# UPC-ViRVIG/DragPoser

Hardware: AMD Instinct MI355X
Metric: frames/sec (6 trackers, 50 iters/frame) (higher is better)
Workload: dtype f32

## Files before the change

dragposer_amd/csrc/dp_w4_impl.h:

```cpp
#pragma once
#ifndef W4_BP
#define W4_BP 0
#endif
#ifndef W4_SKEL
#define W4_SKEL 0
#endif
#ifndef W4_KERNEL
#define W4_KERNEL dp_w4_kernel
#endif
#include "dp_device.h"
#include "dp_w4.h"
#include <utility>

using namespace dpw4;

template <class F, int... I> DEV void static_for_impl(F&& f, std::integer_sequence<int, I...>) { (f(std::integral_constant<int, I>{}), ...); }
template <int N, class F> DEV void static_for(F&& f) { static_for_impl(f, std::make_integer_sequence<int, N>{}); }

constexpr int W4_R = 24;
constexpr int FB_QS = 0;
constexpr int FB_BN = FB_QS + 128;
constexpr int FB_GP = FB_BN + 128;
constexpr int FB_RT = FB_GP + 4 * W4_R;
constexpr int FB_WT = FB_RT + 4 * W4_R;
// ... 297 lines not shown
};
static_assert(sizeof(StepArgs) <= L_ARGS_WORDS * 4 && alignof(StepArgs) <= 16, "StepArgs fits its LDS slot");
DEV void stage_step_args(float* lds, const KArgs& a)
{
    StepArgs* d = (StepArgs*)(lds + L_ARGS);
    d->items = a.items; d->w4img = a.w4img;
    d->z_tgt = a.z_tgt; d->tgt_pos = a.tgt_pos; d->tgt_rot = a.tgt_rot; d->w = a.w;
    d->z = a.z; d->z_pre = a.z_pre; d->pose = a.pose; d->disp = a.disp; d->world_disp = a.world_disp; d->world_rot = a.world_rot;
    d->pos = a.pos; d->rot = a.rot; d->loss = a.loss;
    d->iters = a.iters; d->status = a.status;
    d->n_iter = a.n_iter;
    d->lam_rot = a.lam_rot; d->lam_tmp = a.lam_tmp;
    d->seq = a.seq;
}
template <bool SEQ> DEV decltype(auto) step_args_of(const KArgs& a, const float* lds)
{
    if constexpr (SEQ) {
        int o = L_ARGS;
        asm volatile("" : "+v"(o));
        return *(const StepArgs*)(lds + o);
    } else {
        return (a);
    }
}

DEV int nth_set_bit(unsigned m, int rank)
{
    int pos = 0;
#pragma unroll
    for (int step = 16; step >= 1; step >>= 1) {
        const int c = __popc(m & ((1u << (pos + step)) - 1u));
        pos += c <= rank ? step : 0;
    }
    return pos;
}
struct TRaw {
    bool act;
    int rank, j;
    unsigned plo, phi;
    float p[3], wp, wr, m[9];
};
template <class A> DEV TRaw tracker_fetch(const A& a, bool optimise, int gf, unsigned tmask, int E, int rank, int gf_tgt = -1)
{
    TRaw r;
    r.act = rank < E;
    r.rank = rank;
    const int j = r.act ? nth_set_bit(tmask, rank) : 0;
    r.j = j;
    {
        const auto* it = (const dpl::ItemConst __attribute__((address_space(1)))*)a.items + j;
        r.plo = it->path_lo;
        r.phi = it->path_hi;
    }
    const int row = optimise ? gf * NJ + j : 0;
    const size_t rowt = optimise ? (size_t)(gf_tgt >= 0 ? gf_tgt : gf) * NJ + j : 0;
    const gfloat* p = GM(optimise ? a.tgt_pos : a.w4img) + rowt * 3;
    const gfloat* rm = GM(optimise ? a.tgt_rot : a.w4img) + rowt * 9;
    const gfloat* wv = GM(optimise ? a.w : a.w4img) + (size_t)row * 2;
    r.p[0] = p[0]; r.p[1] = p[1]; r.p[2] = p[2];
    r.wp = wv[0];
    r.wr = wv[1];
#pragma unroll
    for (int k = 0; k < 9; ++k) r.m[k] = rm[k];
    return r;
}
template <class A> DEV TRec tracker_finish(const A& a, float* fb, const TRaw& r, int E, Q4 cur, V3 shift = V3{0.f, 0.f, 0.f})
{
    TRec t;
    t.act = r.act;
    t.rank = r.rank;
    const int j = r.j;
    t.qs = FB_QS + 4 * (j == 0 ? QS_IDENT : j);
    t.wt = FB_WT + 4 * (j == 0 ? WT_TRASH : j);
    t.plo = r.plo;
    t.phi = r.phi;
    t.tp = {0.f, 0.f, 0.f};
    t.qT0 = f2{1.f, 0.f}; t.qT1 = f2{0.f, 0.f};
    t.cgp = t.clp = t.k8 = t.clr8 = 0.f;
    if (t.act) {
        const float invE = 1.f / (float)E;
        t.tp = rot_conj(cur, V3{r.p[0] + shift.x, r.p[1] + shift.y, r.p[2] + shift.z});
        const Q4 qT = quat_mul(Q4{cur.w, -cur.x, -cur.y, -cur.z}, quat_from_rotmat(r.m));
        t.qT0 = f2{qT.w, qT.x}; t.qT1 = f2{qT.y, qT.z};
        t.clp = r.wp * invE * (1.f / 3.f);
        const float clr = a.lam_rot * r.wr * invE * (1.f / 9.f);
        t.cgp = 2.f * t.clp;
        t.k8 = -8.f * clr;
        t.clr8 = 8.f * clr;
        float* ti = fb + FB_TI + r.rank * 4;
        *(f4*)(ti) = f4{t.tp.x, t.tp.y, t.tp.z, t.cgp};
        *(f4*)(ti + 4 * W4_R) = f4{qT.w, qT.x, qT.y, qT.z};
        *(f4*)(ti + 8 * W4_R) = f4{t.k8, t.clp, t.clr8, __int_as_float(j)};
    }
    return t;
}
DEV bool out_of_range(float x) { return !(fabsf(x) <= DP_INPUT_LIMIT); }
DEV bool raw_bad(const TRaw& r)
{
    bool bad = out_of_range(r.p[0]) || out_of_range(r.p[1]) || out_of_range(r.p[2]) || out_of_range(r.wp) || out_of_range(r.wr);
#pragma unroll
    for (int k = 0; k < 9; ++k) bad = bad || out_of_range(r.m[k]);
    return r.act && bad;
}
DEV void raw_neutral(TRaw& r)
{
    r.p[0] = r.p[1] = r.p[2] = 0.f;
    r.wp = r.wr = 0.f;
#pragma unroll
    for (int k = 0; k < 9; ++k) r.m[k] = (k % 4 == 0) ? 1.f : 0.f;
}
DEV unsigned frames_of(unsigned long long votes)
{
    votes |= votes >> 32; votes |= votes >> 16; votes |= votes >> 8; votes |= votes >> 4;
    return (unsigned)votes & 0xFu;
}
DEV float poisoned(bool p, float v) { return p ? __builtin_nanf("") : v; }
template <class A> DEV TRec make_tracker(const A& a, float* fb, int gf, unsigned tmask, int E, int rank, Q4 cur, int gf_tgt = -1, V3 shift = V3{0.f, 0.f, 0.f}, bool neutral = false)
{
    TRaw r = tracker_fetch(a, true, gf, tmask, E, rank, gf_tgt);
    if (neutral) raw_neutral(r);
    return tracker_finish(a, fb, r, E, cur, shift);
}

DEV TRec load_tracker(const KArgs& a, const float* fb, int E, int rank)
{
    TRec t;
    t.act = rank < E;
    t.rank = rank;
    const float* ti = fb + FB_TI + (t.act ? rank : 0) * 4;
    const f4 i0 = *(const f4*)(ti), i1 = *(const f4*)(ti + 4 * W4_R), i2 = *(const f4*)(ti + 8 * W4_R);
    const int j = t.act ? __float_as_int(i2.w) : 0;
    t.qs = FB_QS + 4 * (j == 0 ? QS_IDENT : j);
    t.wt = FB_WT + 4 * (j == 0 ? WT_TRASH : j);
    t.plo = a.items[j].path_lo;
    t.phi = a.items[j].path_hi;
    t.tp = {i0.x, i0.y, i0.z};
    t.cgp = i0.w;
    t.qT0 = f2{i1.x, i1.y}; t.qT1 = f2{i1.z, i1.w};
    t.k8 = i2.x; t.clp = i2.y; t.clr8 = i2.z;
    return t;
}

DEV void lds_store4(float* p, float a, float b, float c, float d)
{
    const unsigned ad = (unsigned)(size_t)p;
    asm volatile("ds_write2_b32 %0, %1, %2 offset1:1\n\tds_write2_b32 %0, %3, %4 offset0:2 offset1:3" : : "v"(ad), "v"(a), "v"(b), "v"(c), "v"(d) : "memory");
}
DEV void lds_store3(float* p, float a, float b, float c)
{
    const unsigned ad = (unsigned)(size_t)p;
    asm volatile("ds_write2_b32 %0, %1, %2 offset1:1\n\tds_write_b32 %0, %3 offset:8" : : "v"(ad), "v"(a), "v"(b), "v"(c) : "memory");
}

struct JOut { f2 q[4], u[3], inv; };
DEV void j_stage(const PairC& c, float* fb, const f4 y01, const f4 y23, JOut& o)
{
    const f2 rq[4] = {f2{y01[0], y01[1]}, f2{y01[2], y01[3]}, f2{y23[0], y23[1]}, f2{y23[2], y23[3]}};
    const f2 nn = rq[0] * rq[0] + rq[1] * rq[1] + rq[2] * rq[2] + rq[3] * rq[3];
#if W4_BP
    const float invA = c.kindA == KIND_DISP ? 1.f : (c.kindA == KIND_IDLE ? 0.f : __builtin_amdgcn_rsqf(nn.x));
    const float invB = c.kindB == KIND_IDLE ? 0.f : __builtin_amdgcn_rsqf(nn.y);
#else
    const float invA = __builtin_amdgcn_rsqf(nn.x);
    const float invB = c.kindB == KIND_DISP ? 1.f : (c.kindB == KIND_IDLE ? 0.f : __builtin_amdgcn_rsqf(nn.y));
#endif
    o.inv = f2{invA, invB};
#pragma unroll
    for (int k = 0; k < 4; ++k) o.q[k] = rq[k] * o.inv;
    const f2 w = o.q[0], vx = o.q[1], vy = o.q[2], vz = o.q[3];
    const f2 tx = vy * c.off[2] - vz * c.off[1], ty = vz * c.off[0] - vx * c.off[2], tz = vx * c.off[1] - vy * c.off[0];
    const f2 cx = vy * tz - vz * ty, cy = vz * tx - vx * tz, cz = vx * ty - vy * tx;
    o.u[0] = c.off[0] + 2.f * (w * tx + cx);
    o.u[1] = c.off[1] + 2.f * (w * ty + cy);
    o.u[2] = c.off[2] + 2.f * (w * tz + cz);
    lds_store4(fb + c.qsA, o.q[0].x, o.q[1].x, o.q[2].x, o.q[3].x);
    lds_store4(fb + c.qsB, o.q[0].y, o.q[1].y, o.q[2].y, o.q[3].y);
    lds_store3(fb + c.bnA, o.u[0].x, o.u[1].x, o.u[2].x);
    lds_store3(fb + c.bnB, o.u[0].y, o.u[1].y, o.u[2].y);
}

DEV void quat_mul_conj_a(f2 a0, f2 a1, f2 b0, f2 b1, f2& o0, f2& o1)
{
    asm("v_pk_mul_f32 %0, %2, %4 op_sel:[1,1] op_sel_hi:[1,0] neg_hi:[0,1]\n\t"
        "v_pk_mul_f32 %1, %2, %5 op_sel:[1,1] op_sel_hi:[1,0] neg_hi:[0,1]\n\t"
        "v_pk_fma_f32 %0, %2, %4, %0 op_sel_hi:[0,1,1]\n\t"
        "v_pk_fma_f32 %1, %2, %5, %1 op_sel_hi:[0,1,1]\n\t"
        "v_pk_fma_f32 %0, %3, %5, %0 op_sel_hi:[0,1,1] neg_hi:[0,1,0]\n\t"
        "v_pk_fma_f32 %1, %3, %4, %1 op_sel_hi:[0,1,1] neg_lo:[0,1,0]\n\t"
        "v_pk_fma_f32 %0, %3, %5, %0 op_sel:[1,1,0] op_sel_hi:[1,0,1]\n\t"
        "v_pk_fma_f32 %1, %3, %4, %1 op_sel:[1,1,0] op_sel_hi:[1,0,1] neg_lo:[0,1,0] neg_hi:[0,1,0]"
        : "=&v"(o0), "=&v"(o1)
        : "v"(a0), "v"(a1), "v"(b0), "v"(b1));
}
DEV void quat_mul_conj_b(f2 a0, f2 a1, f2 b0, f2 b1, f2& o0, f2& o1)
{
    asm("v_pk_mul_f32 %0, %2, %4 op_sel:[1,1] op_sel_hi:[1,0]\n\t"
        "v_pk_mul_f32 %1, %2, %5 op_sel:[1,1] op_sel_hi:[1,0] neg_hi:[0,1]\n\t"
        "v_pk_fma_f32 %0, %2, %4, %0 op_sel_hi:[0,1,1] neg_hi:[0,1,0]\n\t"
        "v_pk_fma_f32 %1, %2, %5, %1 op_sel_hi:[0,1,1] neg_lo:[0,1,0] neg_hi:[0,1,0]\n\t"
        "v_pk_fma_f32 %0, %3, %5, %0 op_sel_hi:[0,1,1] neg_hi:[0,1,0]\n\t"
        "v_pk_fma_f32 %1, %3, %4, %1 op_sel_hi:[0,1,1]\n\t"
        "v_pk_fma_f32 %0, %3, %5, %0 op_sel:[1,1,0] op_sel_hi:[1,0,1]\n\t"
        "v_pk_fma_f32 %1, %3, %4, %1 op_sel:[1,1,0] op_sel_hi:[1,0,1] neg_lo:[0,1,0]"
        : "=&v"(o0), "=&v"(o1)
        : "v"(a0), "v"(a1), "v"(b0), "v"(b1));
}

DEV void t_stage(const TRec& t, float* fb, bool losses)
{
    if (!t.act) return;
    const f4 q0v = *(const f4*)(fb + FB_QS), qtv = *(const f4*)(fb + t.qs), dv = *(const f4*)(fb + FB_QS + 4 * QS_DISP);
    f2 pxy = f2{dv.x, dv.y};
    float pz = dv.z;
    {
        const unsigned plo = t.plo, phi = t.phi;
        f4 bn[MAX_PATH];
#pragma unroll
        for (int k = 0; k < MAX_PATH; ++k) bn[k] = *(const f4*)(fb + FB_BN + 4 * ((k < 6) ? ((plo >> (5 * k)) & 31u) : (phi & 31u)));
#pragma unroll
        for (int k = 0; k < MAX_PATH; ++k) { pxy += f2{bn[k].x, bn[k].y}; pz += bn[k].z; }
    }
    const Q4 q0 = {q0v.x, q0v.y, q0v.z, q0v.w};
    const V3 at = rot_conj(q0, t.tp);
    const f2 exy = pxy - f2{at.x, at.y};
    const float ez = pz - at.z;
    const f2 gpxy = t.cgp * exy;
    const float gpz = t.cgp * ez;
    const V3 e = {exy.x, exy.y, ez}, gp = {gpxy.x, gpxy.y, gpz};
    f2 r0, r1, s0, s1;
    quat_mul_conj_a(f2{q0v.x, q0v.y}, f2{q0v.z, q0v.w}, t.qT0, t.qT1, r0, r1);
    quat_mul_conj_b(r0, r1, f2{qtv.x, qtv.y}, f2{qtv.z, qtv.w}, s0, s1);
    const Q4 s = {s0.x, s0.y, s1.x, s1.y};
    const float k = t.k8 * s.w;
    const float ownx = k * s.x;
    const f2 ownyz = k * s1;
    const V3 own = {ownx, ownyz.x, ownyz.y};
    const V3 ag = cross(at, gp);
    const f2 rtyz = f2{ag.y, ag.z} + ownyz;
    const V3 rt = {ag.x + own.x, rtyz.x, rtyz.y};
    typedef float f3 __attribute__((ext_vector_type(3)));
    *(f3*)(fb + FB_GP + 4 * t.rank) = f3{gp.x, gp.y, gp.z};
    *(f3*)(fb + FB_RT + 4 * t.rank) = f3{rt.x, rt.y, rt.z};
    *(f3*)(fb + t.wt) = f3{own.x, own.y, own.z};
    if (losses)
        *(f2*)(fb + FB_LP + 2 * t.rank) = f2{t.clp * (e.x * e.x + e.y * e.y + e.z * e.z), t.clr8 * (s.x * s.x + s.y * s.y + s.z * s.z)};
}

DEV void g_stage(const PairC& c, const float* fb, const JOut& j, unsigned tmask, int Emax, f4& gyA, f4& gyB)
{
    f2 S[3] = {splat2(0.f), splat2(0.f), splat2(0.f)};
    {
        const float* tab = fb + c.tab;
        f4 g[6];
#pragma unroll
        for (int u = 0; u < 6; ++u) g[u] = *(const f4*)(tab + 4 * u);
#pragma unroll
        for (int u = 0; u < 6; ++u) asm volatile("" : "+v"(g[u]));
#pragma unroll
        for (int u = 0; u < 6; ++u) { S[0] += c.sel[u] * splat2(g[u].x); S[1] += c.sel[u] * splat2(g[u].y); S[2] += c.sel[u] * splat2(g[u].z); }
        if (Emax > 6) {
            unsigned m = tmask;
#pragma unroll
            for (int u = 0; u < 6; ++u) m &= m - 1u;
            for (int e0 = 6; e0 < Emax; ++e0) {
                const f4 ge = *(const f4*)(tab + 4 * e0);
                const int t = __builtin_ctz(m | 0x80000000u);
                m &= m - 1u;
                const f2 sl = f2{(float)((c.subA >> t) & 1u), (float)((c.subB >> t) & 1u)};
                S[0] += sl * splat2(ge.x); S[1] += sl * splat2(ge.y); S[2] += sl * splat2(ge.z);
            }
        }
    }
    f4 wa = *(const f4*)(fb + c.wtA), wb = *(const f4*)(fb + c.wtB);
    asm volatile("" : "+v"(wa), "+v"(wb));
    f2 t0 = j.u[1] * S[2] - j.u[2] * S[1] + c.rho * S[0];
    f2 t1 = j.u[2] * S[0] - j.u[0] * S[2] + c.rho * S[1];
    f2 t2 = j.u[0] * S[1] - j.u[1] * S[0] + c.rho * S[2];
    t0.x += wa.x; t0.y += wb.x; t1.x += wa.y; t1.y += wb.y; t2.x += wa.z; t2.y += wb.z;
    const f2 a0 = t0 + t0, a1 = t1 + t1, a2 = t2 + t2;
    const f2 w = j.q[0], vx = j.q[1], vy = j.q[2], vz = j.q[3];
    const f2 g0 = -(a0 * vx + a1 * vy + a2 * vz);
    const f2 g1 = w * a0 + c.sgn * (a1 * vz - a2 * vy);
    const f2 g2 = w * a1 + c.sgn * (a2 * vx - a0 * vz);
    const f2 g3 = w * a2 + c.sgn * (a0 * vy - a1 * vx);
    const f2 si = j.inv;
    f2 y0 = g0 * si, y1 = g1 * si, y2 = g2 * si, y3 = g3 * si;
#if W4_BP
    if (c.kindA == KIND_DISP) { y0.x = S[0].x; y1.x = S[1].x; y2.x = S[2].x; y3.x = 0.f; }
#else
    if (c.kindB == KIND_DISP) { y0.y = S[0].y; y1.y = S[1].y; y2.y = S[2].y; y3.y = 0.f; }
#endif
    gyA = f4{y0.x, y1.x, y2.x, y3.x};
    gyB = f4{y0.y, y1.y, y2.y, y3.y};
}

struct OutC { int item, kind; f4 sd, mu; unsigned plo, phi; };
DEV void out_consts(const float* oc, int itemA, int kindA, int itemB, int kindB, OutC& oA, OutC& oB)
{
    const f4* t = (const f4*)oc;
    const f4 s0 = t[0], s1 = t[1], m0 = t[2], m1 = t[3], pw = t[4];
    oA.item = itemA; oA.kind = kindA;
    oB.item = itemB; oB.kind = kindB;
    oA.sd = f4{s0.x, s0.z, s1.x, s1.z}; oB.sd = f4{s0.y, s0.w, s1.y, s1.w};
    oA.mu = f4{m0.x, m0.z, m1.x, m1.z}; oB.mu = f4{m0.y, m0.w, m1.y, m1.w};
    oA.plo = __float_as_uint(pw.x); oA.phi = __float_as_uint(pw.y);
    oB.plo = __float_as_uint(pw.z); oB.phi = __float_as_uint(pw.w);
}
template <bool SEQ = false, class A>
DEV void w4_outputs(const A& a, const OutC& oc, float* fb, int gf, bool optimise, Q4 cur, unsigned tmask, bool early, bool pall = false, bool ploss = false)
{
    const int item = oc.item, kind = oc.kind;
    const auto P = [pall](float v) { return poisoned(pall, v); };
    if (item < 0 || kind == KIND_IDLE || kind == KIND_VIRT) return;
    const f4 sd = oc.sd, mu = oc.mu;
    const f4 qv = *(const f4*)(fb + FB_QS + 4 * item);
    const Q4 rq = {qv.x, qv.y, qv.z, qv.w};
    const f4 q0v = *(const f4*)(fb + FB_QS);
    const Q4 qw = quat_mul(cur, Q4{q0v.x, q0v.y, q0v.z, q0v.w});
    const M3 R0 = quat_to_mat(qw);
    if (kind == KIND_DISP) {
        if (a.disp) { gfloat* o = GM(a.disp) + (size_t)gf * 3; o[0] = P(rq.w); o[1] = P(rq.x); o[2] = P(rq.y); }
        if (a.world_disp || SEQ) {
            const V3 wd = mat_vec(R0, V3{rq.w, rq.x, rq.y});
            if (a.world_disp) { gfloat* o = GM(a.world_disp) + (size_t)gf * 3; o[0] = P(wd.x); o[1] = P(wd.y); o[2] = P(wd.z); }
            if (SEQ) { *(f4*)(fb + FB_SWD) = f4{wd.x, wd.y, wd.z, 0.f}; *(f4*)(fb + FB_SD) = f4{rq.w, rq.x, rq.y, 0.f}; }
        }
        return;
    }
    const Q4 q = rq;
    if (a.pose) {
        gfloat* o = GM(a.pose) + (size_t)gf * 88 + 4 * item;
        if (SEQ && kind == KIND_ROOT) {
            o[0] = P((qw.w - a.seq.mean_q0[0]) / a.seq.std_q0[0]); o[1] = P((qw.x - a.seq.mean_q0[1]) / a.seq.std_q0[1]);
            o[2] = P((qw.y - a.seq.mean_q0[2]) / a.seq.std_q0[2]); o[3] = P((qw.z - a.seq.mean_q0[3]) / a.seq.std_q0[3]);
        } else {
            o[0] = P((q.w - mu.x) / sd.x); o[1] = P((q.x - mu.y) / sd.y); o[2] = P((q.y - mu.z) / sd.z); o[3] = P((q.z - mu.w) / sd.w);
        }
    }
    if (a.pos || SEQ) {
        const f4 dv = *(const f4*)(fb + FB_QS + 4 * QS_DISP);
        V3 pr = {dv.x, dv.y, dv.z};
        const unsigned plo = oc.plo, phi = oc.phi;
        f4 bn[MAX_PATH];
#pragma unroll
        for (int k = 0; k < MAX_PATH; ++k) bn[k] = *(const f4*)(fb + FB_BN + 4 * ((k < 6) ? ((plo >> (5 * k)) & 31u) : (phi & 31u)));
#pragma unroll
        for (int k = 0; k < MAX_PATH; ++k) { pr.x += bn[k].x; pr.y += bn[k].y; pr.z += bn[k].z; }
        const V3 pw = mat_vec(R0, pr);
        if (a.pos) { gfloat* o = GM(a.pos) + ((size_t)gf * NJ + item) * 3; o[0] = P(pw.x); o[1] = P(pw.y); o[2] = P(pw.z); }
        if (SEQ) { float* o = fb + FB_SPOS + 3 * item; o[0] = pw.x; o[1] = pw.y; o[2] = pw.z; }
    }
    if (a.rot) {
        M3 M = quat_to_mat(q);
        if (kind == KIND_ROOT) M = {1.f, 0.f, 0.f, 0.f, 1.f, 0.f, 0.f, 0.f, 1.f};
        const M3 G = mat_mat(R0, M);
        gfloat* o = GM(a.rot) + ((size_t)gf * NJ + item) * 9;
        o[0] = P(G.m00); o[1] = P(G.m01); o[2] = P(G.m02); o[3] = P(G.m10); o[4] = P(G.m11); o[5] = P(G.m12); o[6] = P(G.m20); o[7] = P(G.m21); o[8] = P(G.m22);
    }
    if (kind == KIND_ROOT) {
        if (a.world_rot) { gfloat* o = GM(a.world_rot) + (size_t)gf * 4; o[0] = P(qw.w); o[1] = P(qw.x); o[2] = P(qw.y); o[3] = P(qw.z); }
        if (SEQ) *(f4*)(fb + FB_SQW) = f4{qw.w, qw.x, qw.y, qw.z};
        if (optimise && a.loss && early) {
            const f4 es = *(const f4*)(fb + FB_ES);
            gfloat* o = GM(a.loss) + (size_t)gf * 3;
            o[0] = poisoned(ploss, es.x); o[1] = poisoned(ploss, es.y); o[2] = poisoned(ploss, es.z);
        } else if (optimise && a.loss) {
            float lsum_p = 0.f, lsum_r = 0.f, lt = 0.f;
            const int E = min(__popc(tmask), W4_R);
            for (int e0 = 0; e0 < E; ++e0) { const f2 l = *(const f2*)(fb + FB_LP + 2 * e0); lsum_p += l.x; lsum_r += l.y; }
            for (int k = 0; k < LAT; k += 4) {
                const f4 dz = *(const f4*)(fb + FB_ZPRE + k) - *(const f4*)(fb + FB_ZT + k);
                lt += dz.x * dz.x + dz.y * dz.y + dz.z * dz.z + dz.w * dz.w;
            }
            gfloat* o = GM(a.loss) + (size_t)gf * 3;
            o[0] = poisoned(ploss, lsum_p);
            o[1] = poisoned(ploss, lsum_r);
            o[2] = poisoned(ploss, lt * a.lam_tmp * (1.f / 24.f));
        }
    }
}

#ifndef W4_B2_RES_A
#define W4_B2_RES_A 3
#endif
#ifndef W4_B2_RES_V
#define W4_B2_RES_V 2
#endif
#ifndef W4_B2_RES_A_SEQ
#define W4_B2_RES_A_SEQ 1
#endif
template <int NW, bool EARLY, bool SEQ = false, bool LONG = false>
__global__ __launch_bounds__(NW * 64, 1) void W4_KERNEL(const KArgs a)
{
    static_assert(!SEQ || EARLY, "sequences run the reference's while-condition");
    static_assert(W4_B2_RES_A_SEQ >= 1 && W4_B2_RES_A >= 1, "the first resident group of bL2 starts the chain from zero");
    __shared__ __attribute__((aligned(16))) float lds[lds_total<NW>()];

#ifdef DP_PROFILE
    const unsigned long long t_entry = __builtin_amdgcn_s_memtime();
    unsigned long long t_setup[5] = {0, 0, 0, 0, 0};
#define SETUP_STAMP(i) do { __builtin_amdgcn_sched_barrier(0); t_setup[i] = __builtin_amdgcn_s_memtime(); __builtin_amdgcn_sched_barrier(0); } while (0)
#else
#define SETUP_STAMP(i)
#endif
    const int tid = threadIdx.x;
    const int lane = tid & 63;
    const int wave = __builtin_amdgcn_readfirstlane(tid >> 6);
    const int b = lane >> 2, i = lane & 3;
    const int nB = a.n_frames;
    const int f0 = (blockIdx.x * NW + wave) * FPW;
    const bool optimise = (a.mode == 0);

    const int gfi = min(f0 + i, nB - 1);
    const bool fvalid = f0 + i < nB;
    float* fb0 = lds + L_FR + wave * FPW * FB_STRIDE;
    float* fb = fb0 + i * FB_STRIDE;

    constexpr int N_IMG = N_GROUPS * 64, N_LD = (N_IMG + NW * 64 - 1) / (NW * 64);
    static_assert((N_GROUPS - NG_B2) * 256 <= lds_total<NW>() - L_TAB, "the staging area holds the resident groups");
    f4 im[N_LD];
#pragma unroll
    for (int k = 0; k < N_LD; ++k)
        if (tid + k * NW * 64 < N_IMG) im[k] = ((const f4*)a.w4img)[tid + k * NW * 64];
    __builtin_amdgcn_sched_barrier(0);

    typedef unsigned u32_any __attribute__((aligned(1), may_alias));
// ... 253 lines not shown
    const bool clk_on = a.clk != nullptr && blockIdx.x == 0 && wave == 0;
    unsigned long long clk_c0 = 0, clk_r0 = 0;
    if (clk_on) { clk_r0 = __builtin_amdgcn_s_memrealtime(); clk_c0 = __builtin_amdgcn_s_memtime(); }
    int step = 0;
#ifdef DP_SEQ_STAMPS
    unsigned long long sq_t[5] = {0, 0, 0, 0, 0}, sq_p = __builtin_amdgcn_s_memtime();
#define SQ_STAMP(i) do { __builtin_amdgcn_sched_barrier(0); const unsigned long long n_ = __builtin_amdgcn_s_memtime(); sq_t[i] += n_ - sq_p; sq_p = n_; __builtin_amdgcn_sched_barrier(0); } while (0)
#else
#define SQ_STAMP(i)
#endif
    double* adx = (double*)(lds + lds_adx<NW>()) + 2 * wave;
    constexpr bool PK = W4_PACKED_ADAM && !EARLY;
    f2 zP = {0.f, 0.f}, ztP = zP, mP = zP, vP = zP;
    f4 xz = zD;
    const int lane5 = lane & 31, fhalf = lane >> 5;
    if constexpr (PK) { zP = pack_frames(zD); ztP = pack_frames(ztD); }
    do {
    if (LONG) { adx[0] = a.cont.b1t; adx[1] = a.cont.b2t; }
    if (SEQ) {
        const auto& as = step_args_of<SEQ>(a, lds);
        V3 step_shift = {0.f, 0.f, 0.f};
        int gft = step * nB + gfi;
        asm volatile("" : "+v"(gft));
        if (as.seq.tgt_root) {
            const gfloat* rp = GM(as.seq.tgt_root) + (size_t)gft * 3;
            const f4 gpv = *(const f4*)(fb + FB_GPOS);
            step_shift = {rp[0] - gpv.x, rp[1] - gpv.y, rp[2] - gpv.z};
        }
        {
            f4 cvs = *(const f4*)(fb + FB_CUR);
            TRaw rs = tracker_fetch(as, true, gfi, tmask, E, b, gft);
            if (step > 0) zD = zfinD;
            mD = f4{0.f, 0.f, 0.f, 0.f}; vD = mD;
            if (lane < LAT) {
#pragma unroll
                for (int r = 0; r < FPW; ++r) {
                    const int gf = min(f0 + r, nB - 1);
                    ztD[r] = GM(as.z_tgt)[(size_t)step * as.seq.z_tgt_step + (size_t)gf * as.seq.z_tgt_seq + lane];
                }
            }
            bad_state |= bad_tgt;
            {
                bool tb = raw_bad(rs) || out_of_range(step_shift.x) || out_of_range(step_shift.y) || out_of_range(step_shift.z);
                bool nr = rs.act && not_rotation(rs.m);
                for (int base = 16; base < Emax; base += 16) {
                    const TRaw rx = tracker_fetch(as, true, gfi, tmask, E, base + b, gft);
                    tb = tb || raw_bad(rx);
                    nr = nr || (rx.act && not_rotation(rx.m));
                }
                bad_tgt = frames_of(__ballot(tb));
                not_rot = frames_of(__ballot(nr && !tb));
#pragma unroll
                for (int r = 0; r < FPW; ++r) bad_tgt |= (__ballot(lane < LAT && out_of_range(ztD[r])) != 0ull ? 1u : 0u) << r;
                bad_tgt &= ~bad_state;
                not_rot &= ~(bad_state | bad_tgt);
            }
            const bool my_bad = ((bad_state | bad_tgt) >> i) & 1u;
            if (bad_state | bad_tgt) {
                if (my_bad) { raw_neutral(rs); step_shift = V3{0.f, 0.f, 0.f}; }
                if ((bad_state >> i) & 1u) {
                    cvs = f4{1.f, 0.f, 0.f, 0.f};
                    if (b == 0) *(f4*)(fb + FB_CUR) = cvs;
                }
#pragma unroll
                for (int r = 0; r < FPW; ++r) {
                    if ((bad_state >> r) & 1u) zD[r] = 0.f;
                    if (((bad_state | bad_tgt) >> r) & 1u) ztD[r] = zD[r];
                }
            }
            zfinD = zD;
            if (lane < LAT) {
#pragma unroll
                for (int r = 0; r < FPW; ++r) { const float dz = zD[r] - ztD[r]; fb0[r * FB_STRIDE + FB_LT + lane] = dz * dz; }
            }
            const Q4 cur = {cvs.x, cvs.y, cvs.z, cvs.w};
            trk = tracker_finish(as, fb, rs, E, cur, step_shift);
            for (int base = 16; base < Emax; base += 16) make_tracker(as, fb, gfi, tmask, E, base + b, cur, gft, step_shift, my_bad);
            es_prev = 10000000.f; es_act = true; es_iters = 0;
            wave_sync();
        }
    }
    SQ_STAMP(0);
    for (int iter = 0; iter < a.n_iter; ++iter) {
        const bool last = (iter == a.n_iter - 1);
        const f2 adam_t = *(const f2*)(lds + L_TAB + 2 * (LONG ? min(iter, MAX_ITERS - 1) : iter));
        float step = adam_t.x, rbc2s = adam_t.y;
        if constexpr (LONG) {
            if (iter >= MAX_ITERS) adam_beyond(adx, a.cont, step, rbc2s);
        }
        int o = lane;
        asm volatile("" : "+v"(o));
        const f4* w2 = (const f4*)(lds + L_IMG2) + o;

        f4 x = PK ? xz : zD;
#ifdef W4_STAMP_L0
        {
            int t_;
            asm volatile("v_readfirstlane_b32 %0, %1\n\ts_nop 3\n\ts_add_u32 %0, %0, 0" : "=s"(t_) : "v"(x[2]) : "scc");
        }
        STAMP(12);
#endif
        QT(x);
#ifdef W4_STAMP_L0
        { int t_; asm volatile("s_nop 3\n\tv_readfirstlane_b32 %0, %1\n\ts_nop 3\n\ts_add_u32 %0, %0, 0" : "=s"(t_) : "v"(x[3]) : "scc"); }
        STAMP(13);
#endif
        f4 acc0, acc1;
        chain_a<6, 0, 1>(acc0, acc1, x, wL0, bias0T);
        chain_end(acc0, acc1);
#ifdef W4_STAMP_L0
        STAMP(14);
#endif
        const f4 f0D = lrelu_factor(acc0 + acc1);
#ifdef W4_STAMP_L0
        { int t_; asm volatile("v_readfirstlane_b32 %0, %1\n\ts_nop 3\n\ts_add_u32 %0, %0, 0" : "=s"(t_) : "v"(f0D[3]) : "scc"); }
        STAMP(15);
#else
        STAMP(0);
#endif
        x = (acc0 + acc1) * f0D;
        QT(x);
        chain_a<5, 0, 1>(acc0, acc1, x, wL1, bias1T);
        chain_a<5, 8>(acc0, acc1, x, wL1 + 5);
        chain_end(acc0, acc1);
        const f4 f1D = lrelu_factor(acc0 + acc1);
        STAMP(1);
        x = (acc0 + acc1) * f1D;
        QT(x);
        f4 y01, y23;
        {
            f4 pa0, pa1, pb0, pb1;
#if W4_BP
            chain_l2_bp<BP_NG_A, 0>(pa0, pa1, x, wL2A, bias2aT);
            chain_l2_bp<BP_NG_B, 1>(pb0, pb1, x, wL2B, bias2bT);
#else
            chain_a<15, 0, 1>(pa0, pa1, x, wL2A, bias2aT);
            chain_a<15, 0, 1>(pb0, pb1, x, wL2B, bias2bT);
#endif
            chain_end(pa0, pa1);
            y01 = pa0 + pa1;
            y23 = pb0 + pb1;
        }
        __builtin_amdgcn_sched_barrier(0);
        quad_transpose_mfma2(y01, y23, eT);
#if W4_BP
        {
            const f4 yA = y01, yB = y23;
            y01 = f4{yA[0], yB[0], yA[1], yB[1]};
            y23 = f4{yA[2], yB[2], yA[3], yB[3]};
        }
#endif
        STAMP(2);

#ifndef W4_ABLATE_J
        j_stage(pc, fb, y01, y23, jo);
#else
        jo.q[0] = f2{y01[0], y01[1]}; jo.q[1] = f2{y01[2], y01[3]}; jo.q[2] = f2{y23[0], y23[1]}; jo.q[3] = f2{y23[2], y23[3]};
        jo.u[0] = jo.q[0]; jo.u[1] = jo.q[1]; jo.u[2] = jo.q[2]; jo.inv = splat2(1.f);
#endif
        wave_sync();
        STAMP(3);
        if (!optimise) break;
#ifndef W4_ABLATE_T
        t_stage(trk, fb, EARLY || last);
        for (int base = 16; base < Emax; base += 16) t_stage(load_tracker(a, fb, E, base + b), fb, EARLY || last);
#endif
        constexpr int NQ = 8 - B2_RES;
        f4 wq[NQ], wr[8], ws[10];
        if (EARLY || b2_mode != 2) load_w<NQ>(wq, w2 + B2_RES * 64);
        else load_w<NQ>(wq, w2 + 9 * 64);
        __builtin_amdgcn_sched_barrier(0);
        wave_sync();
        STAMP(4);
        unsigned actmask = 0xFu, stopmask = 0u;
        if (EARLY) {
            bool was_act = false, stop_now = false;
            {
                float lp = 0.f, lr = 0.f, lt = 0.f;
                if (Emax <= 8) {
                    f4 l[4];
#pragma unroll
                    for (int k = 0; k < 4; ++k) l[k] = *(const f4*)(fb + FB_LP + 4 * k);
#pragma unroll
                    for (int k = 0; k < 4; ++k) { lp += l[k].x; lr += l[k].y; lp += l[k].z; lr += l[k].w; }
                } else {
                    f4 l[W4_R / 2];
#pragma unroll
                    for (int k = 0; k < W4_R / 2; ++k) l[k] = *(const f4*)(fb + FB_LP + 4 * k);
#pragma unroll
                    for (int k = 0; k < W4_R / 2; ++k) { lp += l[k].x; lr += l[k].y; lp += l[k].z; lr += l[k].w; }
                }
#pragma unroll
                for (int k = 0; k < LAT; k += 4) { const f4 d = *(const f4*)(fb + FB_LT + k); lt += (d.x + d.y) + (d.z + d.w); }
                lt *= a.lam_tmp * (1.f / 24.f);
                const float tot = (lp + lr) + lt;
                const bool cont = (lp > a.stop_eps_pos || lr > a.stop_eps_rot) && (es_prev - tot > a.min_loss_incr) && !last;
                was_act = es_act;
                es_prev = es_act ? tot : es_prev;
                es_iters += es_act ? 1 : 0;
                if (es_act && b == 0) *(f4*)(fb + FB_ES) = f4{lp, lr, lt, 0.f};
                stop_now = es_act && !cont;
                es_act = es_act && cont;
            }
            actmask = (unsigned)__ballot(was_act && b == 0) & 0xFu;
            stopmask = (unsigned)__ballot(stop_now && b == 0) & 0xFu;
        }
        f4 gyA, gyB;
#ifndef W4_ABLATE_G
        g_stage(pc, fb, jo, tmask, Emax, gyA, gyB);
#else
        gyA = f4{jo.q[0].x, jo.q[1].x, jo.q[2].x, jo.q[3].x}; gyB = f4{jo.q[0].y, jo.q[1].y, jo.q[2].y, jo.q[3].y};
#endif
        STAMP(5);

        const auto bl2 = [&](auto skip_tag) {
            constexpr unsigned SK = decltype(skip_tag)::value;
            if constexpr (SK == B2_SKIP_2) {
                static_assert(NQ >= 1 && NQ <= 6, "mode 2 keeps groups 9.. in the first chunk's registers");
                load_w<7 - NQ>(wr, w2 + (9 + NQ) * 64);
                __builtin_amdgcn_sched_barrier(0);
                chain_begin();
                chain_b2<B2_RES_A, 0, 2, SK, true>(acc0, acc1, gyA, gyB, wB2a);
                chain_b2<NQ, 9>(acc0, acc1, gyA, gyB, wq);
                load_w<10>(ws, w2 + 16 * 64);
                __builtin_amdgcn_sched_barrier(0);
                chain_b2<7 - NQ, 9 + NQ>(acc0, acc1, gyA, gyB, wr);
            } else {
                load_w<8, 8, SK>(wr, w2 + 8 * 64);
                __builtin_amdgcn_sched_barrier(0);
                chain_begin();
                chain_b2<B2_RES_A, 0, 2, SK, true>(acc0, acc1, gyA, gyB, wB2a);
                chain_b2<B2_RES_V, B2_RES_A, 0, SK>(acc0, acc1, gyA, gyB, wB2v);
                chain_b2<NQ, B2_RES, 0, SK>(acc0, acc1, gyA, gyB, wq);
                load_w<10>(ws, w2 + 16 * 64);
                __builtin_amdgcn_sched_barrier(0);
                chain_b2<8, 8, 0, SK>(acc0, acc1, gyA, gyB, wr);
            }
            chain_b2<B2_GROUPS_B, ITEMS_A>(acc0, acc1, gyA, gyB, ws);
            chain_end(acc0, acc1);
        };
#ifdef W4_NO_B2_SKIP
        bl2(std::integral_constant<unsigned, 0u>{});
#else
        if constexpr (EARLY) bl2(std::integral_constant<unsigned, 0u>{});
        else {
            if (b2_mode == 0) bl2(std::integral_constant<unsigned, 0u>{});
            else if (b2_mode == 1) bl2(std::integral_constant<unsigned, B2_SKIP_1>{});
            else bl2(std::integral_constant<unsigned, B2_SKIP_2>{});
        }
#endif
        x = (acc0 + acc1) * f1D;
        QT(x);
        STAMP(6);
        chain_a<15, 0, 2>(acc0, acc1, x, wB1);
        chain_end(acc0, acc1);
        x = (acc0 + acc1) * f0D;
        QT(x);
        STAMP(7);
        chain3_v_zero<5>(acc0, acc1, x, wz);
        chain_end(acc0, acc1);
        __builtin_amdgcn_sched_barrier(0);
        f4 g = {0.f, 0.f, 0.f, 0.f};
        f2 gP = {0.f, 0.f};
        if constexpr (PK) gP = add_halves_packed(acc0 + acc1) + a.ctmp * (zP - ztP);
        else g = add_halves(acc0 + acc1) + a.ctmp * (zD - ztD);
        STAMP(8);
        if (PK && DBG_DUMP && a.dbg && iter == 0 && lane5 < LAT) {
            int ld = lane5;
            asm volatile("" : "+v"(ld));
#pragma unroll
            for (int r = 0; r < 2; ++r)
                if (f0 + r + 2 * fhalf < nB) a.dbg[(size_t)(f0 + r + 2 * fhalf) * DBG_STRIDE + DBG_GZ + ld] = gP[r];
        }
        if (!PK && DBG_DUMP && a.dbg && iter == 0 && lane < LAT) {
            int ld = lane;
            asm volatile("" : "+v"(ld));
#pragma unroll
            for (int r = 0; r < FPW; ++r)
                if (f0 + r < nB) a.dbg[(size_t)(f0 + r) * DBG_STRIDE + DBG_GZ + ld] = g[r];
        }
#ifdef W4_ABLATE_ADAM
        if constexpr (PK) { zP = zP - 1e-6f * gP; xz = unpack_frames(zP, xz); }
        else zD = zD - 1e-6f * g;
#else
        if constexpr (PK) {
            if (last && lane5 < LAT) {
#pragma unroll
                for (int r = 0; r < 2; ++r) fb0[(r + 2 * fhalf) * FB_STRIDE + FB_ZPRE + lane5] = zP[r];
            }
            mP = mP + a.one_m_b1 * (gP - mP);
            vP = vP * a.beta2 + a.one_m_b2 * (gP * gP);
            const f2 den = f2{__builtin_amdgcn_sqrtf(vP.x), __builtin_amdgcn_sqrtf(vP.y)} * rbc2s + a.eps;
            zP = zP - step * (mP * f2{__builtin_amdgcn_rcpf(den.x), __builtin_amdgcn_rcpf(den.y)});
            xz = unpack_frames(zP, xz);
        } else if (!EARLY) {
            if (last && lane < LAT) {
#pragma unroll
                for (int r = 0; r < FPW; ++r) fb0[r * FB_STRIDE + FB_ZPRE + lane] = zD[r];
            }
            mD = mD + a.one_m_b1 * (g - mD);
            vD = vD * a.beta2 + a.one_m_b2 * (g * g);
            const f4 den = f4{__builtin_amdgcn_sqrtf(vD.x), __builtin_amdgcn_sqrtf(vD.y), __builtin_amdgcn_sqrtf(vD.z),
                              __builtin_amdgcn_sqrtf(vD.w)} * rbc2s + a.eps;
            zD = zD - step * (mD * f4{__builtin_amdgcn_rcpf(den.x), __builtin_amdgcn_rcpf(den.y), __builtin_amdgcn_rcpf(den.z),
                                      __builtin_amdgcn_rcpf(den.w)});
        } else {
            const f4 mN = mD + a.one_m_b1 * (g - mD);
            const f4 vN = vD * a.beta2 + a.one_m_b2 * (g * g);
            const f4 den = f4{__builtin_amdgcn_sqrtf(vN.x), __builtin_amdgcn_sqrtf(vN.y), __builtin_amdgcn_sqrtf(vN.z),
                              __builtin_amdgcn_sqrtf(vN.w)} * rbc2s + a.eps;
            const f4 zN = zD - step * (mN * f4{__builtin_amdgcn_rcpf(den.x), __builtin_amdgcn_rcpf(den.y), __builtin_amdgcn_rcpf(den.z),
                                               __builtin_amdgcn_rcpf(den.w)});
#pragma unroll
            for (int r = 0; r < FPW; ++r) {
                if ((actmask >> r) & 1u) {
                    if ((stopmask >> r) & 1u) {
                        if (lane < LAT) fb0[r * FB_STRIDE + FB_ZPRE + lane] = zD[r];
                        zfinD[r] = zN[r];
                    } else {
                        zD[r] = zN[r]; mD[r] = mN[r]; vD[r] = vN[r];
                        const float dz = zN[r] - ztD[r];
                        if (lane < LAT) fb0[r * FB_STRIDE + FB_LT + lane] = dz * dz;
                    }
                }
            }
        }
#endif
#ifdef W4_STAMP_L0
        { int t_; asm volatile("v_readfirstlane_b32 %0, %1\n\ts_nop 3\n\ts_add_u32 %0, %0, 0" : "=s"(t_) : "v"(PK ? xz[3] : zD[3]) : "scc"); }
#endif
        STAMP(9);
#ifdef DP_PROFILE
        if (iter == 0) prof.t[18] = prof.prev - mt0;
        if (iter == 1) prof.t[19] = prof.prev - mt0 - prof.t[18];
#endif
        if (EARLY && ((unsigned)__ballot(es_act && b == 0) & 0xFu) == 0u) break;
    }
#ifdef DP_PROFILE
    prof.t[16] = __builtin_amdgcn_s_memrealtime() - rt0;
    prof.t[17] = __builtin_amdgcn_s_memtime() - mt0;
#endif
    SQ_STAMP(1);
    if constexpr (PK) { if (optimise) zD = xz; }
    const auto& ae = step_args_of<SEQ>(a, lds);
    asm volatile("" : "+s"(bad_state), "+s"(bad_tgt), "+s"(not_rot));
    const unsigned pois_z = bad_state | bad_tgt, pois_all = bad_state | ((EARLY || ae.n_iter == 1) ? 0u : bad_tgt);
    int row0 = SEQ ? step * nB : 0;
    int gfo = row0 + gfi;
    int lane_e = lane, item_eA = pc.itemA, item_eB = pc.itemB, f0_e = f0, gfi_e = gfi;
    if (SEQ) {
        asm volatile("" : "+v"(gfo)); asm volatile("" : "+s"(row0));
        asm volatile("" : "+v"(lane_e), "+v"(item_eA), "+v"(item_eB), "+v"(gfi_e));
        asm volatile("" : "+s"(f0_e));
    }
    if (lane < LAT) {
#pragma unroll
        for (int r = 0; r < FPW; ++r) {
            if (!optimise) fb0[r * FB_STRIDE + FB_ZPRE + lane] = zD[r];
            fb0[r * FB_STRIDE + FB_ZT + lane] = ztD[r];
        }
    }
    wave_sync();
// ... 100 lines not shown
```

Before: 35.29 million.

## Issue LDS reads for tracker and gradient stages earlier to hide latency

Splits the tracker and gradient stages into separate read and compute phases. The tracker's quaternion and bone-offset LDS reads can now be issued inside the joint stage, right after the matching stores, and the gradient table and weight reads can be issued before the weight-chunk global loads. Which of these early reads are enabled is chosen per template variant through a bitmask macro. The aim is to overlap LDS latency with arithmetic and wave sync waits, at the cost of more live registers and relying on ordering within a wave for correctness.

```diff
diff --git a/dragposer_amd/csrc/dp_w4_impl.h b/dragposer_amd/csrc/dp_w4_impl.h
--- a/dragposer_amd/csrc/dp_w4_impl.h
+++ b/dragposer_amd/csrc/dp_w4_impl.h
@@ -473,8 +473,23 @@
     asm volatile("ds_write2_b32 %0, %1, %2 offset1:1\n\tds_write_b32 %0, %3 offset:8" : : "v"(ad), "v"(a), "v"(b), "v"(c) : "memory");
 }
 
+#ifndef W4_EARLY_READS
+#define W4_EARLY_READS 7
+#endif
+struct TRd { f4 q0v, qtv, dv, bn[MAX_PATH]; };
+DEV void t_reads_q(const TRec& t, const float* fb, TRd& r)
+{
+    r.q0v = *(const f4*)(fb + FB_QS); r.qtv = *(const f4*)(fb + t.qs); r.dv = *(const f4*)(fb + FB_QS + 4 * QS_DISP);
+}
+DEV void t_reads_bn(const TRec& t, const float* fb, TRd& r)
+{
+    const unsigned plo = t.plo, phi = t.phi;
+#pragma unroll
+    for (int k = 0; k < MAX_PATH; ++k) r.bn[k] = *(const f4*)(fb + FB_BN + 4 * ((k < 6) ? ((plo >> (5 * k)) & 31u) : (phi & 31u)));
+}
+
 struct JOut { f2 q[4], u[3], inv; };
-DEV void j_stage(const PairC& c, float* fb, const f4 y01, const f4 y23, JOut& o)
+template <bool TREADS> DEV void j_stage(const PairC& c, float* fb, const f4 y01, const f4 y23, JOut& o, const TRec& t, TRd& tr)
 {
     const f2 rq[4] = {f2{y01[0], y01[1]}, f2{y01[2], y01[3]}, f2{y23[0], y23[1]}, f2{y23[2], y23[3]}};
     const f2 nn = rq[0] * rq[0] + rq[1] * rq[1] + rq[2] * rq[2] + rq[3] * rq[3];
@@ -489,15 +504,27 @@
 #pragma unroll
     for (int k = 0; k < 4; ++k) o.q[k] = rq[k] * o.inv;
     const f2 w = o.q[0], vx = o.q[1], vy = o.q[2], vz = o.q[3];
+    if constexpr (TREADS) {
+        lds_store4(fb + c.qsA, o.q[0].x, o.q[1].x, o.q[2].x, o.q[3].x);
+        lds_store4(fb + c.qsB, o.q[0].y, o.q[1].y, o.q[2].y, o.q[3].y);
+        t_reads_q(t, fb, tr);
+        __builtin_amdgcn_sched_barrier(0);
+    }
     const f2 tx = vy * c.off[2] - vz * c.off[1], ty = vz * c.off[0] - vx * c.off[2], tz = vx * c.off[1] - vy * c.off[0];
     const f2 cx = vy * tz - vz * ty, cy = vz * tx - vx * tz, cz = vx * ty - vy * tx;
     o.u[0] = c.off[0] + 2.f * (w * tx + cx);
     o.u[1] = c.off[1] + 2.f * (w * ty + cy);
     o.u[2] = c.off[2] + 2.f * (w * tz + cz);
-    lds_store4(fb + c.qsA, o.q[0].x, o.q[1].x, o.q[2].x, o.q[3].x);
-    lds_store4(fb + c.qsB, o.q[0].y, o.q[1].y, o.q[2].y, o.q[3].y);
+    if constexpr (!TREADS) {
+        lds_store4(fb + c.qsA, o.q[0].x, o.q[1].x, o.q[2].x, o.q[3].x);
+        lds_store4(fb + c.qsB, o.q[0].y, o.q[1].y, o.q[2].y, o.q[3].y);
+    }
     lds_store3(fb + c.bnA, o.u[0].x, o.u[1].x, o.u[2].x);
     lds_store3(fb + c.bnB, o.u[0].y, o.u[1].y, o.u[2].y);
+    if constexpr (TREADS) {
+        t_reads_bn(t, fb, tr);
+        __builtin_amdgcn_sched_barrier(0);
+    }
 }
 
 DEV void quat_mul_conj_a(f2 a0, f2 a1, f2 b0, f2 b1, f2& o0, f2& o1)
@@ -527,30 +554,32 @@
         : "v"(a0), "v"(a1), "v"(b0), "v"(b1));
 }
 
-DEV void t_stage(const TRec& t, float* fb, bool losses)
-{
-    if (!t.act) return;
-    const f4 q0v = *(const f4*)(fb + FB_QS), qtv = *(const f4*)(fb + t.qs), dv = *(const f4*)(fb + FB_QS + 4 * QS_DISP);
+template <bool AHEAD> DEV void t_finish(const TRec& t, float* fb, bool losses, TRd& rd)
+{
+    if constexpr (!AHEAD) {
+        if (!t.act) return;
+    }
+    const f4 q0v = rd.q0v, qtv = rd.qtv;
+    const Q4 q0 = {q0v.x, q0v.y, q0v.z, q0v.w};
+    V3 at = rot_conj(q0, t.tp);
+    f2 r0, r1, s0, s1;
+    quat_mul_conj_a(f2{q0v.x, q0v.y}, f2{q0v.z, q0v.w}, t.qT0, t.qT1, r0, r1);
+    quat_mul_conj_b(r0, r1, f2{qtv.x, qtv.y}, f2{qtv.z, qtv.w}, s0, s1);
+    if constexpr (AHEAD) {
+        asm volatile("" : "+v"(rd.dv), "+v"(rd.bn[0]), "+v"(rd.bn[1]), "+v"(rd.bn[2]), "+v"(rd.bn[3]), "+v"(rd.bn[4]), "+v"(rd.bn[5]), "+v"(rd.bn[6]),
+                          "+v"(s0), "+v"(s1), "+v"(at.x), "+v"(at.y), "+v"(at.z));
+        static_assert(MAX_PATH == 7, "the statement above names every bone read");
+    }
+    const f4 dv = rd.dv;
     f2 pxy = f2{dv.x, dv.y};
     float pz = dv.z;
-    {
-        const unsigned plo = t.plo, phi = t.phi;
-        f4 bn[MAX_PATH];
-#pragma unroll
-        for (int k = 0; k < MAX_PATH; ++k) bn[k] = *(const f4*)(fb + FB_BN + 4 * ((k < 6) ? ((plo >> (5 * k)) & 31u) : (phi & 31u)));
-#pragma unroll
-        for (int k = 0; k < MAX_PATH; ++k) { pxy += f2{bn[k].x, bn[k].y}; pz += bn[k].z; }
-    }
-    const Q4 q0 = {q0v.x, q0v.y, q0v.z, q0v.w};
-    const V3 at = rot_conj(q0, t.tp);
+#pragma unroll
+    for (int k = 0; k < MAX_PATH; ++k) { pxy += f2{rd.bn[k].x, rd.bn[k].y}; pz += rd.bn[k].z; }
     const f2 exy = pxy - f2{at.x, at.y};
     const float ez = pz - at.z;
     const f2 gpxy = t.cgp * exy;
     const float gpz = t.cgp * ez;
     const V3 e = {exy.x, exy.y, ez}, gp = {gpxy.x, gpxy.y, gpz};
-    f2 r0, r1, s0, s1;
-    quat_mul_conj_a(f2{q0v.x, q0v.y}, f2{q0v.z, q0v.w}, t.qT0, t.qT1, r0, r1);
-    quat_mul_conj_b(r0, r1, f2{qtv.x, qtv.y}, f2{qtv.z, qtv.w}, s0, s1);
     const Q4 s = {s0.x, s0.y, s1.x, s1.y};
     const float k = t.k8 * s.w;
     const float ownx = k * s.x;
@@ -560,21 +589,41 @@
     const f2 rtyz = f2{ag.y, ag.z} + ownyz;
     const V3 rt = {ag.x + own.x, rtyz.x, rtyz.y};
     typedef float f3 __attribute__((ext_vector_type(3)));
+    if constexpr (AHEAD) {
+        if (!t.act) return;
+    }
     *(f3*)(fb + FB_GP + 4 * t.rank) = f3{gp.x, gp.y, gp.z};
     *(f3*)(fb + FB_RT + 4 * t.rank) = f3{rt.x, rt.y, rt.z};
     *(f3*)(fb + t.wt) = f3{own.x, own.y, own.z};
     if (losses)
         *(f2*)(fb + FB_LP + 2 * t.rank) = f2{t.clp * (e.x * e.x + e.y * e.y + e.z * e.z), t.clr8 * (s.x * s.x + s.y * s.y + s.z * s.z)};
 }
-
-DEV void g_stage(const PairC& c, const float* fb, const JOut& j, unsigned tmask, int Emax, f4& gyA, f4& gyB)
+DEV void t_stage(const TRec& t, float* fb, bool losses)
+{
+    if (!t.act) return;
+    TRd rd;
+    t_reads_q(t, fb, rd);
+    t_reads_bn(t, fb, rd);
+    t_finish<false>(t, fb, losses, rd);
+}
+
+struct GRd { f4 g[6], wa, wb; };
+template <bool WAB> DEV void g_reads(const PairC& c, const float* fb, GRd& r)
+{
+    const float* tab = fb + c.tab;
+#pragma unroll
+    for (int u = 0; u < 6; ++u) r.g[u] = *(const f4*)(tab + 4 * u);
+    if constexpr (WAB) {
+        __builtin_amdgcn_sched_barrier(0);
+        r.wa = *(const f4*)(fb + c.wtA); r.wb = *(const f4*)(fb + c.wtB);
+    }
+}
+template <bool WAB> DEV void g_stage(const PairC& c, const float* fb, const JOut& j, unsigned tmask, int Emax, GRd& r, f4& gyA, f4& gyB)
 {
     f2 S[3] = {splat2(0.f), splat2(0.f), splat2(0.f)};
     {
         const float* tab = fb + c.tab;
-        f4 g[6];
-#pragma unroll
-        for (int u = 0; u < 6; ++u) g[u] = *(const f4*)(tab + 4 * u);
+        f4* const g = r.g;
 #pragma unroll
         for (int u = 0; u < 6; ++u) asm volatile("" : "+v"(g[u]));
 #pragma unroll
@@ -592,7 +641,8 @@
             }
         }
     }
-    f4 wa = *(const f4*)(fb + c.wtA), wb = *(const f4*)(fb + c.wtB);
+    if constexpr (!WAB) { r.wa = *(const f4*)(fb + c.wtA); r.wb = *(const f4*)(fb + c.wtB); }
+    f4 wa = r.wa, wb = r.wb;
     asm volatile("" : "+v"(wa), "+v"(wb));
     f2 t0 = j.u[1] * S[2] - j.u[2] * S[1] + c.rho * S[0];
     f2 t1 = j.u[2] * S[0] - j.u[0] * S[2] + c.rho * S[1];
@@ -1152,26 +1202,41 @@
 #endif
         STAMP(2);
 
+        constexpr int ER = W4_EARLY_READS & (W4_BP ? 7 : (EARLY ? 1 : 3));
+        constexpr bool G_WAB = (ER & 1) != 0, WQ_LATE = (ER & 2) != 0, T_EARLY = (ER & 4) != 0;
+        TRd trd;
 #ifndef W4_ABLATE_J
-        j_stage(pc, fb, y01, y23, jo);
+        j_stage<T_EARLY>(pc, fb, y01, y23, jo, trk, trd);
 #else
         jo.q[0] = f2{y01[0], y01[1]}; jo.q[1] = f2{y01[2], y01[3]}; jo.q[2] = f2{y23[0], y23[1]}; jo.q[3] = f2{y23[2], y23[3]};
         jo.u[0] = jo.q[0]; jo.u[1] = jo.q[1]; jo.u[2] = jo.q[2]; jo.inv = splat2(1.f);
+        if constexpr (T_EARLY) { t_reads_q(trk, fb, trd); t_reads_bn(trk, fb, trd); }
 #endif
         wave_sync();
         STAMP(3);
         if (!optimise) break;
 #ifndef W4_ABLATE_T
-        t_stage(trk, fb, EARLY || last);
+        if constexpr (T_EARLY) t_finish<true>(trk, fb, EARLY || last, trd);
+        else t_stage(trk, fb, EARLY || last);
         for (int base = 16; base < Emax; base += 16) t_stage(load_tracker(a, fb, E, base + b), fb, EARLY || last);
 #endif
         constexpr int NQ = 8 - B2_RES;
         f4 wq[NQ], wr[8], ws[10];
-        if (EARLY || b2_mode != 2) load_w<NQ>(wq, w2 + B2_RES * 64);
-        else load_w<NQ>(wq, w2 + 9 * 64);
-        __builtin_amdgcn_sched_barrier(0);
+        const auto load_wq = [&] {
+            if (EARLY || b2_mode != 2) load_w<NQ>(wq, w2 + B2_RES * 64);
+            else load_w<NQ>(wq, w2 + 9 * 64);
+            __builtin_amdgcn_sched_barrier(0);
+        };
+        if constexpr (!WQ_LATE) load_wq();
         wave_sync();
         STAMP(4);
+        GRd grd;
+        if constexpr (WQ_LATE) {
+#ifndef W4_ABLATE_G
+            g_reads<G_WAB>(pc, fb, grd);
+#endif
+            if constexpr (!EARLY) load_wq();
+        }
         unsigned actmask = 0xFu, stopmask = 0u;
         if (EARLY) {
             bool was_act = false, stop_now = false;
@@ -1204,10 +1269,12 @@
             }
             actmask = (unsigned)__ballot(was_act && b == 0) & 0xFu;
             stopmask = (unsigned)__ballot(stop_now && b == 0) & 0xFu;
+            if constexpr (WQ_LATE) load_wq();
         }
         f4 gyA, gyB;
 #ifndef W4_ABLATE_G
-        g_stage(pc, fb, jo, tmask, Emax, gyA, gyB);
+        if constexpr (!WQ_LATE) g_reads<G_WAB>(pc, fb, grd);
+        g_stage<G_WAB>(pc, fb, jo, tmask, Emax, grd, gyA, gyB);
 #else
         gyA = f4{jo.q[0].x, jo.q[1].x, jo.q[2].x, jo.q[3].x}; gyB = f4{jo.q[0].y, jo.q[1].y, jo.q[2].y, jo.q[3].y};
 #endif
```

Result: faster. 35.85 million (median of 6 runs) (+1.6%).
